# CWBudde/go-pocket-tts

Measured on AMD Instinct MI355X. Metric: synthesized audio sec/sec (xRT), higher is better.
Workload: dtype bf16; 1 GPU; b64_10s_bf16: 64 utterances/GPU x 125 frames (10.0 s each), 25-token prompt + 125-frame voice state, greedy (temperature 0), hipGraph-captured AR step, Mimi decode to 24 kHz PCM written to host; batch_per_gpu=64, frames=125, weights=BF16, kv=bf16, checkpoint=synthetic, shapes of tts_b6369a24 (seed 1234)

## Files before the change

go-pocket-tts_amd/csrc/flow_cluster.hip:

```cpp
#include <hip/hip_ext.h>

#include "../../include/ptts.h"
#include "common.h"
#include "kernels.h"
#include "device_util.h"

namespace ptts {

typedef __bf16 fc_bf16x8 __attribute__((ext_vector_type(8)));
typedef __bf16 fc_bf16x2 __attribute__((ext_vector_type(2)));
typedef float fc_f32x2 __attribute__((ext_vector_type(2)));
typedef float fc_f32x4 __attribute__((ext_vector_type(4)));
typedef unsigned fc_u32x4 __attribute__((ext_vector_type(4)));

constexpr int FC_C = 512;
constexpr int FC_RB = 2048, FC_CMASK = 127;
constexpr unsigned FC_SPIN_LIMIT = 1u << 15;
constexpr int FC_FAULT_WORD = 32 * kFlowClusterMaxTiles;

union FcFrag {
    fc_bf16x8 v;
    uint4 q;
};

__device__ __forceinline__ void fc_split2(float a, float b, unsigned& hi, unsigned& lo) {
    fc_f32x2 f = {a, b};
    fc_bf16x2 h = __builtin_convertvector(f, fc_bf16x2);
    fc_f32x2 r = f - __builtin_convertvector(h, fc_f32x2);
    fc_bf16x2 l = __builtin_convertvector(r, fc_bf16x2);
    hi = *reinterpret_cast<unsigned*>(&h);
    lo = *reinterpret_cast<unsigned*>(&l);
}

__device__ __forceinline__ void fc_stage(unsigned char* Xh, unsigned char* Xl, int wave, int lane, const float4 (&xr)[2]) {
#pragma unroll
    for (int j = 0; j < 2; j++) {
        const int k = (lane + 64 * j) * 4;
        unsigned h01, l01, h23, l23;
// ... 8 lines not shown
template <typename RS>
__device__ __forceinline__ bool fc_sweep(RS rs, int row_off, int lane, unsigned tag, float4 (&xr)[2]) {
    fc_u32x4 g0 = {0u, 0u, 0u, 0u}, g1 = g0, g2 = g0, g3 = g0;
    bool got = true;
    const int voff = row_off + lane * 32;
    const int watch = row_off + ((lane >> 1) * 16 + 6 + 8 * (lane & 1)) * 8;
    for (unsigned spins = 0;; spins++) {
        asm volatile("" ::: "memory");
        const fc_u32x4 w = __builtin_amdgcn_raw_buffer_load_b128(rs, watch, 0, 16);
        if (__all(w[1] == tag && w[3] == tag)) {
            asm volatile("" ::: "memory");
            g0 = __builtin_amdgcn_raw_buffer_load_b128(rs, voff, 0, 16);
            g1 = __builtin_amdgcn_raw_buffer_load_b128(rs, voff + 16, 0, 16);
            g2 = __builtin_amdgcn_raw_buffer_load_b128(rs, voff + 2048, 0, 16);
            g3 = __builtin_amdgcn_raw_buffer_load_b128(rs, voff + 2064, 0, 16);
            const bool ok = g0[1] == tag && g0[3] == tag && g1[1] == tag && g1[3] == tag && g2[1] == tag && g2[3] == tag && g3[1] == tag && g3[3] == tag;
            if (__all(ok)) break;
        }
        if (spins > FC_SPIN_LIMIT) { got = false; g0 = g1 = g2 = g3 = fc_u32x4{0u, 0u, 0u, 0u}; break; }
        __builtin_amdgcn_s_sleep(8);
    }
    xr[0] = make_float4(__uint_as_float(g0[0]), __uint_as_float(g0[2]), __uint_as_float(g1[0]), __uint_as_float(g1[2]));
    xr[1] = make_float4(__uint_as_float(g2[0]), __uint_as_float(g2[2]), __uint_as_float(g3[0]), __uint_as_float(g3[2]));
    return got;
}

template <typename RS>
__device__ __forceinline__ void fc_publish(RS rs, int voff, unsigned tag, const float (&v)[4]) {
    const fc_u32x4 a = {__float_as_uint(v[0]), tag, __float_as_uint(v[1]), tag}, b = {__float_as_uint(v[2]), tag, __float_as_uint(v[3]), tag};
    __builtin_amdgcn_raw_buffer_store_b128(a, rs, voff, 0, 16);
    __builtin_amdgcn_raw_buffer_store_b128(b, rs, voff + 16, 0, 16);
}

constexpr int FC_ROWS = kFlowClusterRows;
constexpr int FC_THREADS = 64 * (4 + FC_ROWS);
constexpr int FC_TILE_GRANULES = 2 * 16 * FC_C;

template <bool STAMP>
__global__ __launch_bounds__(FC_THREADS) void k_flow_cluster(FlowClusterArgs a) {
#define FC_STAMP(i) do { if (STAMP && lane == 0) a.stamps[blockIdx.x * 64 + (i)] = __builtin_amdgcn_s_memrealtime(); } while (0)
    __shared__ __attribute__((aligned(16))) unsigned char Xh[16 * FC_RB];
    __shared__ __attribute__((aligned(16))) unsigned char Xl[16 * FC_RB];
    const int tid = threadIdx.x, lane = tid & 63, wave = __builtin_amdgcn_readfirstlane(tid >> 6);
    const int cb = blockIdx.x & 7, tile = blockIdx.x >> 3;
    const int m0 = tile * FC_ROWS;
    unsigned* const sync = a.sync + tile * 32;
    const unsigned base = __builtin_amdgcn_readfirstlane(__hip_atomic_load(sync, __ATOMIC_RELAXED, __HIP_MEMORY_SCOPE_AGENT));
    auto rs = __builtin_amdgcn_make_buffer_rsrc(a.xbuf + (size_t)tile * FC_TILE_GRANULES, 0, FC_TILE_GRANULES * 8, 0x00020000);
    constexpr int BUF1 = 16 * FC_C * 8;

    if (wave < 4) {
        const int cg = wave, q = lane >> 4, i16 = lane & 15;
        const bool s_ok = i16 < FC_ROWS && m0 + i16 < a.rows;
        const int64_t srow = s_ok ? m0 + i16 : 0;
        const int scol = cb * 64 + cg * 16 + q * 4;
        const int pub_off = i16 * (FC_C * 8) + scol * 8;
        const int64_t wfrag = ((int64_t)(cb * 4 + cg) * 16) * 64 + lane;
        uint4 w[16];
        {
            const uint4* s0 = reinterpret_cast<const uint4*>(a.w0[0]) + wfrag;
#pragma unroll
            for (int i = 0; i < 16; i++) w[i] = s0[i * 64];
        }
        float4 res = *reinterpret_cast<const float4*>(a.fx_in + srow * FC_C + scol);
        auto product = [&](float (&acc)[4]) {
#pragma unroll
            for (int ss = 0; ss < 4; ss++) {
                fc_f32x4 acc_h = {0.f, 0.f, 0.f, 0.f}, acc_l = {0.f, 0.f, 0.f, 0.f};
#pragma unroll
                for (int s = 0; s < 4; s++) {
                    const int off = i16 * FC_RB + (((q * 4 + s) ^ i16) << 4) + ss * 256;
                    FcFrag xh, xl, wv;
                    xh.q = *reinterpret_cast<const uint4*>(&Xh[off]);
                    xl.q = *reinterpret_cast<const uint4*>(&Xl[off]);
                    wv.q = w[ss * 4 + s];
                    acc_h = __builtin_amdgcn_mfma_f32_16x16x32_bf16(wv.v, xh.v, acc_h, 0, 0, 0);
                    acc_l = __builtin_amdgcn_mfma_f32_16x16x32_bf16(wv.v, xl.v, acc_l, 0, 0, 0);
                }
                const fc_f32x4 accv = acc_h + acc_l;
                if (ss == 0) { acc[0] = accv[0]; acc[1] = accv[1]; acc[2] = accv[2]; acc[3] = accv[3]; }
                else { acc[0] += accv[0]; acc[1] += accv[1]; acc[2] += accv[2]; acc[3] += accv[3]; }
            }
        };
        auto next_weights = [&](const void* wt) {
            const uint4* sw = reinterpret_cast<const uint4*>(wt) + wfrag;
#pragma unroll
            for (int i = 0; i < 16; i++) w[i] = sw[i * 64];
        };
        if (wave == 0) FC_STAMP(0);
#pragma unroll 1
        for (int r = 0; r < a.depth; r++) {
            const int rn = min(r + 1, a.depth - 1);
            const void* const pw2 = a.w2[r]; const void* const pw0n = a.w0[rn];
            const float* const pb0 = a.b0[r]; const float* const pb2 = a.b2[r];
            asm volatile("" ::"s"(pw2), "s"(pw0n), "s"(pb0), "s"(pb2));
            const float4 bias0 = *reinterpret_cast<const float4*>(pb0 + scol);
            float acc[4];
            __syncthreads();
            if (wave == 0) FC_STAMP(1 + 4 * r);
            product(acc);
            next_weights(pw2);
            if (STAMP && wave == 0 && r == 2) { if (acc[0] == 1.2345e-30f) FC_STAMP(60); FC_STAMP(56); }
            {
                const float h[4] = {silu1(acc[0] + bias0.x), silu1(acc[1] + bias0.y), silu1(acc[2] + bias0.z), silu1(acc[3] + bias0.w)};
                if (STAMP && wave == 0 && r == 2) { if (h[0] == 1.2345e-30f) FC_STAMP(60); FC_STAMP(58); }
                if (s_ok && !(a.inject && tile == 0 && cb == 7 && r == a.inject - 1)) fc_publish(rs, BUF1 + pub_off, base + 2 * r + 1, h);
            }
            if (STAMP && wave == 0 && r == 2) FC_STAMP(57);
            if (wave == 0) FC_STAMP(2 + 4 * r);
            const float4 bias2 = *reinterpret_cast<const float4*>(pb2 + scol);
            const float4 gate = *reinterpret_cast<const float4*>(a.ada + srow * a.ldmod + (int64_t)(r * 3 + 2) * FC_C + scol);
            __syncthreads();
            if (wave == 0) FC_STAMP(3 + 4 * r);
            product(acc);
            next_weights(pw0n);
            res.x = res.x + gate.x * (acc[0] + bias2.x);
            res.y = res.y + gate.y * (acc[1] + bias2.y);
            res.z = res.z + gate.z * (acc[2] + bias2.z);
            res.w = res.w + gate.w * (acc[3] + bias2.w);
            if (s_ok) {
                if (r + 1 < a.depth) {
                    const float v[4] = {res.x, res.y, res.z, res.w};
                    fc_publish(rs, pub_off, base + 2 * r + 2, v);
                } else *reinterpret_cast<float4*>(a.fx_out + srow * FC_C + scol) = res;
            }
            if (wave == 0) FC_STAMP(4 + 4 * r);
        }
        if (cb == 0 && tid == 0) __hip_atomic_store(sync, base + 2u * (unsigned)a.depth, __ATOMIC_RELAXED, __HIP_MEMORY_SCOPE_AGENT);
        if (wave == 0) FC_STAMP(31);
    } else {
        const int row = wave - 4;
        const bool row_ok = m0 + row < a.rows;
        const int64_t mrow = row_ok ? m0 + row : 0;
        const int kc0 = lane * 4, kc1 = (lane + 64) * 4;
        const int sweep_off = row * (FC_C * 8);
        unsigned fault = 0;
#pragma unroll 1
        for (int r = 0; r < a.depth; r++) {
            if (row_ok) {
                float4 xr[2];
                const float* lnw = a.ln_w[r]; const float* lnb = a.ln_b[r];
                const float* shift = a.ada + mrow * a.ldmod + (int64_t)(r * 3) * FC_C; const float* scale = shift + FC_C;
                const float4 lw0 = *reinterpret_cast<const float4*>(lnw + kc0), lw1 = *reinterpret_cast<const float4*>(lnw + kc1);
                const float4 lb0 = *reinterpret_cast<const float4*>(lnb + kc0), lb1 = *reinterpret_cast<const float4*>(lnb + kc1);
                const float4 lc0 = *reinterpret_cast<const float4*>(scale + kc0), lc1 = *reinterpret_cast<const float4*>(scale + kc1);
                const float4 lh0 = *reinterpret_cast<const float4*>(shift + kc0), lh1 = *reinterpret_cast<const float4*>(shift + kc1);
                if (r == 0) {
                    xr[0] = *reinterpret_cast<const float4*>(a.fx_in + mrow * FC_C + kc0);
                    xr[1] = *reinterpret_cast<const float4*>(a.fx_in + mrow * FC_C + kc1);
                } else if (!fc_sweep(rs, sweep_off, lane, base + 2 * r, xr)) fault = 1;
                if (wave == 4) FC_STAMP(32 + 4 * r);
                fc_f32x2 s2 = {0.f, 0.f};
#pragma unroll
                for (int j = 0; j < 2; j++) s2 += fc_f32x2{xr[j].x, xr[j].z} + fc_f32x2{xr[j].y, xr[j].w};
                const float rk = __builtin_amdgcn_rcpf((float)FC_C);
                const float mean = wave_sum_dpp(s2.x + s2.y) * rk;
                const fc_f32x2 m2 = {mean, mean};
                fc_f32x2 v2 = {0.f, 0.f};
#pragma unroll
                for (int j = 0; j < 2; j++) {
                    const fc_f32x2 da = fc_f32x2{xr[j].x, xr[j].y} - m2, db = fc_f32x2{xr[j].z, xr[j].w} - m2;
                    v2 += da * da + db * db;
                }
                const float inv_std = __builtin_amdgcn_rsqf(wave_sum_dpp(v2.x + v2.y) * rk + a.eps[r]);
                const fc_f32x2 is2 = {inv_std, inv_std};
#pragma unroll
                for (int j = 0; j < 2; j++) {
                    const float4 lw = j ? lw1 : lw0, lb = j ? lb1 : lb0, lc = j ? lc1 : lc0, lh = j ? lh1 : lh0;
                    fc_f32x2 oa = (fc_f32x2{xr[j].x, xr[j].y} - m2) * is2, ob = (fc_f32x2{xr[j].z, xr[j].w} - m2) * is2;
                    oa = oa * fc_f32x2{lw.x, lw.y} + fc_f32x2{lb.x, lb.y};
                    ob = ob * fc_f32x2{lw.z, lw.w} + fc_f32x2{lb.z, lb.w};
                    const fc_f32x2 one = {1.0f, 1.0f};
                    oa = oa * (fc_f32x2{lc.x, lc.y} + one) + fc_f32x2{lh.x, lh.y};
                    ob = ob * (fc_f32x2{lc.z, lc.w} + one) + fc_f32x2{lh.z, lh.w};
                    xr[j] = make_float4(oa.x, oa.y, ob.x, ob.y);
                }
                fc_stage(Xh, Xl, row, lane, xr);
            }
            if (wave == 4) FC_STAMP(33 + 4 * r);
            __syncthreads();
            if (row_ok) {
                float4 xr[2];
                if (!fc_sweep(rs, BUF1 + sweep_off, lane, base + 2 * r + 1, xr)) fault = 1;
                if (wave == 4) FC_STAMP(34 + 4 * r);
                fc_stage(Xh, Xl, row, lane, xr);
            }
            if (wave == 4) FC_STAMP(35 + 4 * r);
            __syncthreads();
        }
        if (fault && lane == 0) atomicOr(a.sync + FC_FAULT_WORD, 1u);
    }
#undef FC_STAMP
}

bool flow_cluster_supported(const FlowClusterArgs& a, int C) {
    if (C != FC_C || a.rows <= 0 || a.rows > kFlowClusterMaxTiles * kFlowClusterRows || a.depth <= 0 || a.depth > FC_MAX_DEPTH || a.ldmod % 4 != 0 || !a.xbuf || !a.sync) return false;
    if (!aligned16(a.fx_in) || !aligned16(a.fx_out) || !aligned16(a.ada)) return false;
    for (int r = 0; r < a.depth; r++)
        if (!a.w0[r] || !a.w2[r] || !a.b0[r] || !a.b2[r] || !a.ln_w[r] || !a.ln_b[r] || !aligned16(a.b0[r]) || !aligned16(a.b2[r]) || !aligned16(a.ln_w[r]) || !aligned16(a.ln_b[r])) return false;
    return true;
}

bool flow_cluster_fits(int rows, int device) {
    int cus = 0, per_cu = 0;
    if (hipDeviceGetAttribute(&cus, hipDeviceAttributeMultiprocessorCount, device) != hipSuccess || cus <= 0) return false;
    if (hipOccupancyMaxActiveBlocksPerMultiprocessor(&per_cu, k_flow_cluster<false>, FC_THREADS, 0) != hipSuccess || per_cu <= 0) { (void)hipGetLastError(); return false; }
    return 8 * ((rows + FC_ROWS - 1) / FC_ROWS) <= cus * per_cu;
}

void launch_flow_cluster(const FlowClusterArgs& a, hipStream_t stream, hipEvent_t ev0, hipEvent_t ev1) {
    note_launch("k_flow_cluster");
    const dim3 grid(8 * ((a.rows + FC_ROWS - 1) / FC_ROWS));
    if (a.stamps) hipLaunchKernelGGL(k_flow_cluster<true>, grid, dim3(FC_THREADS), 0, stream, a);
    else if (ev0) hipExtLaunchKernelGGL(k_flow_cluster<false>, grid, dim3(FC_THREADS), 0, stream, ev0, ev1, 0, a);
    else hipLaunchKernelGGL(k_flow_cluster<false>, grid, dim3(FC_THREADS), 0, stream, a);
}

}
```

go-pocket-tts_amd/csrc/kernels.h:

```cpp
#pragma once

#include <hip/hip_runtime.h>
#include <atomic>
#include <cstdint>
#include <map>
#include <string>
#include <vector>

namespace ptts {

struct RowMap {
    int64_t ld = 0;
    int64_t rows_per_batch = 0;
    int64_t batch_stride = 0;
};

enum AOp : int { AOP_NONE = 0, AOP_ELU = 1 };
enum Epi : int {
    EPI_NONE = 0,
    EPI_GELU,
    EPI_SILU,
    EPI_ELU,
    EPI_RESADD,
    EPI_SCALE_RESADD,
// ... 264 lines not shown
};
struct RowLinArgs {
    const float* x = nullptr; RowMap xmap;
    const float* ln_w = nullptr; const float* ln_b = nullptr; float eps = 1e-5f;
    const void* img = nullptr;
    float* y = nullptr; RowMap ymap;
    const float* rope_cos = nullptr; const float* rope_sin = nullptr; int rope_cols = 0, rope_pos0 = 0, rope_rows_per_seg = 0;
    int M = 0, N = 0, K = 0;
};
bool mimi_rowlin_supported(const RowLinArgs& a);
void launch_mimi_rowlin(const RowLinArgs& a, hipStream_t stream);
bool mimi_ffn_supported(const FfnArgs& a);
void launch_mimi_ffn(const FfnArgs& a, hipStream_t stream);

constexpr int FC_MAX_DEPTH = 8;
struct FlowClusterArgs {
    const float* fx_in = nullptr; float* fx_out = nullptr;
    const float* ada = nullptr; int64_t ldmod = 0;
    int rows = 0, depth = 0;
    float eps[FC_MAX_DEPTH] = {};
    const float* ln_w[FC_MAX_DEPTH] = {}; const float* ln_b[FC_MAX_DEPTH] = {};
    const void* w0[FC_MAX_DEPTH] = {}; const float* b0[FC_MAX_DEPTH] = {};
    const void* w2[FC_MAX_DEPTH] = {}; const float* b2[FC_MAX_DEPTH] = {};
    unsigned long long* xbuf = nullptr;
    unsigned long long* stamps = nullptr;
    int inject = 0;
    unsigned* sync = nullptr;
};
constexpr int kFlowClusterRows = 12;
constexpr int kFlowClusterMaxTiles = (kStepMaxRows + kFlowClusterRows - 1) / kFlowClusterRows;
constexpr size_t kFlowClusterTileBytes = (size_t)2 * 16 * 512 * 8;
constexpr size_t kFlowClusterSyncBytes = (size_t)(32 * kFlowClusterMaxTiles + 32) * 4;
inline size_t flow_cluster_xbuf_bytes(int rows) { return (size_t)((rows + kFlowClusterRows - 1) / kFlowClusterRows) * kFlowClusterTileBytes; }
bool flow_cluster_fits(int rows, int device);
bool flow_cluster_supported(const FlowClusterArgs& a, int C);
void launch_flow_cluster(const FlowClusterArgs& a, hipStream_t stream, hipEvent_t ev0 = nullptr, hipEvent_t ev1 = nullptr);

struct StepState {
    int32_t* kv_len;
    int32_t* active;
    int32_t* step;
    int32_t* countdown;
    int32_t* n_frames;
    int32_t* eos_step;
    int32_t* max_steps;
    int32_t* frames_after_eos;
    float*   eos_threshold;
    int32_t* n_active;
    int32_t* broke;
};
struct StepChain {
    const void* w_in; const float* b_in; float* x; int32_t d_in;
    const void* w_pj; const float* b_pj; float* fx; int32_t d_pj;
    const float* bos; float* x0; int32_t w_bf16; int32_t ok;
};
struct StepFinish {
    StepState s;
    const float* eos_logit;
    float* latents;
    int64_t lat_stride;
    int32_t ldim;
    StepChain ch;
};
struct StepOpenLinears {
    const void* w_in = nullptr; const float* b_in = nullptr; int d_in = 0; float* x = nullptr;
    const void* w_pj = nullptr; const float* b_pj = nullptr; int d_pj = 0; float* fx = nullptr;
    int w_bf16 = 0;
};
bool step_open_mfma_ok(const StepOpenLinears& lin, int ldim);
void launch_step_begin(const StepState& s, const float* latents, int64_t lat_stride, const float* bos, const float* noise, int64_t noise_stride,
                       int ldim, int b, float* in32, float* x0, const StepOpenLinears* lin, hipStream_t stream);
void launch_step_finish(const StepState& s, const float* frame, const float* eos_logit, int ldim, int b, float* latents,
                        int64_t lat_stride, hipStream_t stream);
struct NoiseSpec { uint64_t seed; float sigma; int32_t rows; };
void launch_noise_fill(const NoiseSpec* spec_dev, int n_slots, int max_rows, float* out, int64_t out_stride, int ldim, hipStream_t stream);
struct GatherTable { struct Row { int32_t src_row, dst_off, nf, T; }; Row rows[128]; };
void launch_gather_frames(const GatherTable& t, int n, const float* stage, int64_t row_stride, float* dst, int ld, hipStream_t stream);
void launch_readback_i32(const int32_t* a, int na, const int32_t* b, int nb, int32_t* host, hipStream_t stream);
struct SlotAdmit { int32_t slot, max_steps, frames_after_eos; float eos_threshold; int32_t kv_len, pre_len; const void* pre_k; const void* pre_v; };
void launch_slot_admit(const StepState& s, int32_t* pre_len, const void** pre_k, const void** pre_v, const SlotAdmit* dev, int n, hipStream_t stream);
void launch_slot_retire(const StepState& s, const int32_t* slots_dev, int n, hipStream_t stream);
void launch_fill_i32(int32_t* p, int32_t v, int n, hipStream_t stream);
void launch_add_i32(int32_t* p, const int32_t* inc, int n, hipStream_t stream);

void launch_enc_head(const float* pcm, const void* w, int w_bf16, const float* b, int64_t L, int C, int k, float* out, int64_t ldo, hipStream_t stream);
int enc_ds_splits(int M, int N, int K);
void launch_enc_downsample(const float* A, int64_t lda, const void* W, int w_bf16, const float* bias, int M, int N, int K, float* partial, float* out,
                           hipStream_t stream);

void launch_bct_to_btc(const float* in, int b, int c, int t, float* out, int out_pad_rows, hipStream_t stream);
void launch_btc_to_bct(const float* in, int in_pad_rows, int b, int c, int t, float* out, hipStream_t stream);

}
```

go-pocket-tts_amd/csrc/runtime.cpp:

```cpp
#include "runtime.h"

#include <chrono>

#include <algorithm>
#include <cmath>

namespace ptts {

static RowMap flat(int64_t ld) { return RowMap{ld, 0, 0}; }
static RowMap seg(int64_t ld, int64_t rows_per_batch, int64_t batch_stride) { return RowMap{ld, rows_per_batch, batch_stride}; }

static GemmArgs mk(const Model& m, const float* A, RowMap am, const Lin& l, float* C, RowMap cm, int M) {
    GemmArgs g;
    g.A = A; g.amap = am;
    g.W = m.arena + l.w; g.w_bf16 = l.bf16; g.ldw = l.in;
    g.Wt = l.wt == NONE ? nullptr : m.arena + l.wt;
    g.wt_i8 = l.wt_i8; g.wscale = m.at<float>(l.wscale);
    g.bias = m.at<float>(l.b);
    g.C = C; g.cmap = cm;
    g.M = M; g.N = l.out; g.K = l.in;
    return g;
}
static LnArgs mkln(const Model& m, const float* x, RowMap xm, const Norm& n, float* y, int64_t ldy, int rows) {
    LnArgs a;
// ... 219 lines not shown
    b->vcache.ensure(kvbytes);
    PTTS_HIP(hipMemsetAsync(b->kcache.p, 0, kvbytes, m.stream));
    PTTS_HIP(hipMemsetAsync(b->vcache.p, 0, kvbytes, m.stream));
    b->state_i32.ensure((9 * B + 1) * sizeof(int32_t));
    b->state_f32.ensure(B * sizeof(float));
    int32_t* s = b->state_i32.as<int32_t>();
    b->st.kv_len = s; b->st.active = s + B; b->st.step = s + 2 * B; b->st.countdown = s + 3 * B;
    b->st.n_frames = s + 4 * B; b->st.eos_step = s + 5 * B; b->st.max_steps = s + 6 * B;
    b->st.frames_after_eos = s + 7 * B; b->st.broke = s + 8 * B; b->st.n_active = s + 9 * B;
    b->st.eos_threshold = b->state_f32.as<float>();
    b->kv_len_host.assign(B, 0);
    b->pre_k.ensure((size_t)B * sizeof(void*)); b->pre_v.ensure((size_t)B * sizeof(void*)); b->pre_len.ensure((size_t)B * sizeof(int32_t));
    b->pre_k_host.assign(B, nullptr); b->pre_v_host.assign(B, nullptr); b->pre_len_host.assign(B, 0);
    const size_t f = sizeof(float);
    const int NA = d.ada_all.out;
    b->in_raw.ensure(B * d.ldim * f); b->in32.ensure(B * d.ldim * f);
    b->x.ensure(B * d.d_model * f); b->xn.ensure(B * std::max(d.d_model, d.flow_dim) * f);
    b->qkv.ensure(B * 3 * d.d_model * f); b->attn.ensure(B * d.d_model * f);
    b->ff.ensure(B * d.ffn * f); b->last.ensure(B * d.d_model * f); b->eos.ensure(B * f);
    b->sy.ensure(B * d.flow_dim * f); b->ada.ensure(B * NA * f);
    b->fx.ensure(B * d.flow_dim * f); b->fh.ensure(B * d.flow_dim * f); b->fh2.ensure(B * d.flow_dim * f);
    b->cur.ensure(B * d.ldim * f);
    b->partial.ensure((size_t)16 * B * std::max(d.d_model, d.flow_dim) * f);
    b->latents.ensure(B * b->max_steps * d.ldim * f);
    {
        StepFinish sf{b->st, b->eos.as<float>(), b->latents.as<float>(), (int64_t)b->max_steps * d.ldim, (int32_t)d.ldim, StepChain{}};
        StepOpenLinears lin;
        b->chain_ok = open_linears(*b, lin) && step_open_mfma_ok(lin, d.ldim) && ((int64_t)b->max_steps * d.ldim) % 2 == 0 &&
                      (lin.w_bf16 != 0) == (d.final_linear.bf16 != 0 || d.final_linear.wt_i8 != 0);
        b->fx2.ensure(B * d.flow_dim * f); b->cur2.ensure(B * d.ldim * f);
        StepFinish sf2[2] = {sf, sf};
        sf2[0].ch = StepChain{lin.w_in, lin.b_in, lin.x, lin.d_in, lin.w_pj, lin.b_pj, b->fx2.as<float>(), lin.d_pj, m.at<float>(d.bos), b->cur2.as<float>(), lin.w_bf16, b->chain_ok ? 1 : 0};
        sf2[1].ch = StepChain{lin.w_in, lin.b_in, lin.x, lin.d_in, lin.w_pj, lin.b_pj, b->fx.as<float>(), lin.d_pj, m.at<float>(d.bos), b->cur.as<float>(), lin.w_bf16, b->chain_ok ? 1 : 0};
        b->fin_dev.ensure(sizeof sf2);
        h2d(b->fin_dev.p, sf2, sizeof sf2, m.stream);
    }
    {
        const char* sw = getenv("PTTS_FLOW_CLUSTER");
        const bool off = sw && sw[0] == '0';
        bool ok = !off && !m.fc_disabled.load() && d.flow_dim == 512 && d.flow_depth > 0 && d.flow_depth <= FC_MAX_DEPTH && n_slots <= kStepMaxRows &&
                  flow_cluster_fits(n_slots, m.device);
        for (int r = 0; ok && r < d.flow_depth; r++) {
            const auto& rb = d.rb[r];
            for (const Lin* l : {&rb.mlp0, &rb.mlp2}) ok = ok && l->in == 512 && l->out == 512 && l->bf16 && !l->wt_i8 && l->wt != NONE && l->b != NONE;
            ok = ok && rb.ln.w != NONE && rb.ln.b != NONE && rb.ln.d == 512;
        }
        b->fc_ok = ok;
        if (ok) {
            b->fc_xbuf.ensure(flow_cluster_xbuf_bytes(n_slots)); b->fc_sync.ensure(kFlowClusterSyncBytes);
            PTTS_HIP(hipMemsetAsync(b->fc_xbuf.p, 0, flow_cluster_xbuf_bytes(n_slots), m.stream));
            PTTS_HIP(hipMemsetAsync(b->fc_sync.p, 0, kFlowClusterSyncBytes, m.stream));
            if (getenv("PTTS_FC_STAMPS")) { b->fc_stamps.ensure((size_t)8 * kFlowClusterMaxTiles * 64 * 8); PTTS_HIP(hipMemsetAsync(b->fc_stamps.p, 0, (size_t)8 * kFlowClusterMaxTiles * 64 * 8, m.stream)); }
        }
    }
    {
        const char* sw = getenv("PTTS_TALL");
        bool ok = !(sw && sw[0] == '0') && n_slots >= kTallMinRows && (d.d_model == 512 || d.d_model == 1024) && d.ffn % 128 == 0;
        for (int l = 0; ok && l < d.n_layers; l++) {
            const auto& L = d.layers[l];
            for (const Lin* li : {&L.in_proj, &L.l1, &L.l2}) ok = ok && li->bf16 && !li->wt_i8 && li->wt != NONE && li->out % 4 == 0;
            ok = ok && L.in_proj.in == d.d_model && L.l1.in == d.d_model && L.l1.out == d.ffn && L.l2.in == d.ffn && L.l2.out == d.d_model;
            ok = ok && L.n1.w != NONE && L.n1.b != NONE && L.n2.w != NONE && L.n2.b != NONE;
        }
        b->tall_ok = ok;
        if (ok) { b->tp_a.ensure(2 * B * d.d_model * sizeof(uint16_t)); b->tp_f.ensure(2 * B * d.ffn * sizeof(uint16_t)); }
    }
    PTTS_HIP(hipHostMalloc((void**)&b->n_active_pinned, sizeof(int32_t) * (size_t)(2 + 2 * B), hipHostMallocDefault));
    PTTS_HIP(hipHostMalloc((void**)&b->rows_pinned, sizeof(PcmRow) * std::max<size_t>((size_t)B, 1), hipHostMallocDefault));
    batch_reset(*b);
    return b.release();
}

void batch_reset(Batch& b) {
    b.opened = false;
    hipStream_t s = b.m->stream;
    const int B = b.B;
    launch_fill_i32(b.st.kv_len, 0, B, s);
    b.kv_bound = 0;
    launch_fill_i32(b.st.active, 1, B, s);
    launch_fill_i32(b.st.step, 0, B, s);
// ... 300 lines not shown
    ln.x = x; ln.xmap = flat(l.in); ln.eps = in.eps; ln.rows = M; ln.d = l.in;
    if (in.norm && in.affine) { ln.w = m.at<float>(in.norm->w); ln.b = m.at<float>(in.norm->b); }
    ln.shift = in.shift; ln.scale = in.scale; ln.ldmod = in.ldmod;
    ln.partial = in.pend.partial; ln.splitk = in.pend.splitk; ln.pstride = in.pend.pstride; ln.pbias = in.pend.bias;
    float* y = in.y_out ? in.y_out : b.xn.as<float>();
    ln.y = y; ln.ldy = l.in;
    if (in.pend.partial) {
        launch_layernorm(ln, m.stream);
        if (in.x_out && in.x_out != x) PTTS_HIP(hipMemcpyAsync(in.x_out, x, (size_t)M * l.in * sizeof(float), hipMemcpyDeviceToDevice, m.stream));
    } else launch_layernorm(ln, m.stream);
    GemmArgs g2 = mk(m, y, flat(l.in), l, C, flat(ldc), M);
    g2.epi = epi; g2.addvec = addvec; g2.R = R; g2.alpha = alpha;
    step_gemm(m, g2);
    return false;
}

static bool open_linears(Batch& b, StepOpenLinears& lin) {
    Model& m = *b.m;
    const Desc& d = m.d;
    const int ld = d.ldim;
    if (!(ld <= 64 && ld % 4 == 0 && d.input_linear.in == ld && d.input_proj.in == ld && d.input_linear.bf16 == d.input_proj.bf16)) return false;
    lin.w_in = m.arena + d.input_linear.w; lin.b_in = m.at<float>(d.input_linear.b); lin.d_in = d.input_linear.out; lin.x = b.x.as<float>();
    lin.w_pj = m.arena + d.input_proj.w; lin.b_pj = m.at<float>(d.input_proj.b); lin.d_pj = d.input_proj.out; lin.fx = b.fx.as<float>();
    lin.w_bf16 = d.input_linear.bf16;
    return true;
}

void flow_cluster_recover(Batch& b) {
    hipStream_t s = b.m->stream;
    (void)hipStreamSynchronize(s);
    (void)hipMemsetAsync(b.fc_xbuf.p, 0, flow_cluster_xbuf_bytes(b.B), s);
    (void)hipMemsetAsync(b.fc_sync.p, 0, kFlowClusterSyncBytes, s);
    (void)hipStreamSynchronize(s);
    b.fc_ok = false;
    for (auto& set : b.graphs) for (auto& row : set) for (hipGraphExec_t& g : row) if (g) { (void)hipGraphExecDestroy(g); g = nullptr; }
    for (auto& gs : b.graph_steps) gs[0] = gs[1] = 0;
    b.opened = false;
    b.m->fc_disabled.store(true);
    b.m->fc_fallbacks.fetch_add(1);
}
void flow_cluster_fault(Batch& b) {
    flow_cluster_recover(b);
    throw FlowClusterFault(PTTS_ENODEVICE, "ptts-hip: the flow net's in-launch hand-off timed out (k_flow_cluster); the steps concerned are re-issued as launches");
}

void step_open(Batch& b) {
    Model& m = *b.m;
    const Desc& d = m.d;
    const int ld = d.ldim;
    const int64_t ls = (int64_t)b.max_steps * ld;
    StepOpenLinears lin;
    const bool ok = open_linears(b, lin);
    b.opened = ok;
    b.par = 0;
    launch_step_begin(b.st, b.latents.as<float>(), ls, m.at<float>(d.bos), b.has_noise ? b.noise.as<float>() : nullptr, ls, ld, b.B,
                      b.in32.as<float>(), b.cur.as<float>(), ok ? &lin : nullptr, m.stream);
}

bool step_core(Batch& b, int lsd, bool opened, bool fuse_finish, bool chain) {
    bool finished = false;
    b.opened = false;
    if (!opened) b.par = 0;
    Model& m = *b.m;
    const Desc& d = m.d;
    hipStream_t s = m.stream;
    const int B = b.B, D = d.d_model, C = d.flow_dim;
    const bool kvb = m.opts.kv == PTTS_KV_BF16;
// ... 127 lines not shown
            ln.partial = pend.partial; ln.splitk = pend.splitk; ln.pstride = pend.pstride; ln.pbias = pend.bias;
            launch_layernorm(ln, s);
            step_gemm(m, mk(m, last, flat(D), d.out_eos, b.eos.as<float>(), flat(1), B));
        }
    }
    b.tail_fused = tail_fused;
    finished = step_flow(b, lsd, opened, fuse_finish, chain);
    if (!b.capturing) b.kv_bound++;
    return finished;
}

static bool step_flow(Batch& b, int lsd, bool opened, bool fuse_finish, bool chain) {
    bool finished = false;
    Model& m = *b.m;
    const Desc& d = m.d;
    const int B = b.B, D = d.d_model, C = d.flow_dim, NA = d.ada_all.out;
    hipStream_t s = m.stream;
    const bool tail_fused = b.tail_fused;
    float* last = b.last.as<float>();
    float* sy = b.sy.as<float>();
    const float* tc = m.tcomb.at(lsd)->as<float>();
    float* ada = b.ada.as<float>();
    float* fx = b.fx_now();
    float* fh2 = b.fh2.as<float>();
    float* cur = b.cur_now();
    for (int i = 0; i < lsd; i++) {
        if (i > 0 || !tail_fused) {
            GemmArgs gc = mk(m, last, flat(D), d.cond_embed, sy, flat(C), B);
            gc.epi = EPI_SILU; gc.addvec = tc + (size_t)i * C;
            step_gemm(m, gc);
        }
        step_gemm(m, mk(m, sy, flat(C), d.ada_all, ada, flat(NA), B));
        if (i > 0 || !opened) step_gemm(m, mk(m, cur, flat(d.ldim), d.input_proj, fx, flat(C), B));
        bool clustered = false;
        if (b.fc_ok) {
            FlowClusterArgs fa;
            fa.fx_in = fx; fa.fx_out = fx; fa.ada = ada; fa.ldmod = NA; fa.rows = B; fa.depth = d.flow_depth;
            for (int r = 0; r < d.flow_depth; r++) {
                const auto& rb = d.rb[r];
                fa.eps[r] = rb.ln.eps; fa.ln_w[r] = m.at<float>(rb.ln.w); fa.ln_b[r] = m.at<float>(rb.ln.b);
                fa.w0[r] = m.arena + rb.mlp0.wt; fa.b0[r] = m.at<float>(rb.mlp0.b);
                fa.w2[r] = m.arena + rb.mlp2.wt; fa.b2[r] = m.at<float>(rb.mlp2.b);
            }
            fa.xbuf = b.fc_xbuf.as<unsigned long long>(); fa.sync = b.fc_sync.as<unsigned>();
            if (b.fc_stamps.p) fa.stamps = b.fc_stamps.as<unsigned long long>();
            if (m.fc_inject && !b.capturing) { fa.inject = m.fc_inject; m.fc_inject = 0; }
            if (flow_cluster_supported(fa, C)) {
                launch_flow_cluster(fa, s);
                clustered = true;
            }
        }
        for (int r = 0; !clustered && r < d.flow_depth; r++) {
            const auto& rb = d.rb[r];
            FusedIn in;
            in.norm = &rb.ln; in.eps = rb.ln.eps;
            in.shift = ada + (size_t)r * 3 * C; in.scale = in.shift + C; in.ldmod = NA;
            step_fused_linear(b, fx, in, rb.mlp0, fh2, C, B, EPI_SILU, nullptr, nullptr, 1.0f);
            GemmArgs g2 = mk(m, fh2, flat(C), rb.mlp2, fx, flat(C), B);
            g2.R = fx; g2.epi = EPI_GATE_RESADD; g2.gate = ada + (size_t)r * 3 * C + 2 * C; g2.ldg = NA;
            step_gemm(m, g2);
        }
        FusedIn fin;
        fin.affine = false; fin.eps = 1e-6f;
        fin.shift = ada + (size_t)d.flow_depth * 3 * C; fin.scale = fin.shift + C; fin.ldmod = NA;
        if (fuse_finish && i == lsd - 1) {
            fin.finish = b.fin_dev.as<StepFinish>() + b.par;
            if (chain && b.chain_ok) {
                fin.chain = true;
                fin.chain_noise = b.has_noise ? b.noise.as<float>() : nullptr;
                fin.chain_noise_stride = (int64_t)b.max_steps * d.ldim;
            }
        }
        bool chained = false;
        finished = step_fused_linear(b, fx, fin, d.final_linear, cur, d.ldim, B, EPI_AXPY, nullptr, cur, 1.0f / (float)lsd, nullptr, &chained);
        if (chained) { b.opened = true; b.par ^= 1; }
    }
    return finished;
}

void step_flow_again(Batch& b, int lsd) {
    b.opened = false; b.par = 0;
    (void)step_flow(b, lsd, false, false, false);
}

void mimi_setup(Model& m, MimiWs& w, int B, int T) {
    const Desc& d = m.d;
    w.B = B; w.T = T;
    const int C = d.mimi_dim, S = d.up_stride, T1 = T * S, F = d.mimi_ffn;
    w.P0 = d.init_k - 1;
    w.Ls[0] = T1; w.Ps[0] = 1;
    for (int j = 0; j < 3; j++) {
        w.Ls[j + 1] = w.Ls[j] * d.strides[j];
        int need_next = j < 2 ? 1 : d.final_k - 1;
// ... 933 lines not shown
```

go-pocket-tts_amd/csrc/runtime.h:

```cpp
#pragma once

#include <atomic>
#include <functional>

#include "kernels.h"
#include "model.h"
#include "row_ring.h"
#include "dsp_spec.h"
#include "host_rows.h"

namespace ptts {

struct DevBuf {
    void* p = nullptr;
    size_t n = 0;
    DevBuf() = default;
    DevBuf(const DevBuf&) = delete;
    DevBuf& operator=(const DevBuf&) = delete;
    ~DevBuf() { release(); }
    void release() {
        if (p) (void)hipFree(p);
        p = nullptr;
        n = 0;
    }
// ... 96 lines not shown
struct PackedRows {
    std::vector<size_t> bytes, off;
    char* base = nullptr;
    PackedRows(Model& m, WorkSlot slot, std::vector<size_t> row_bytes, const bool* skip = nullptr) : bytes(std::move(row_bytes)), off(bytes.size()) {
        base = m.work(slot, std::max<size_t>(pack_rows(bytes.data(), skip, (int)bytes.size(), off.data()), kRowAlign)).as<char>();
    }
    char* row(int i) const { return base + off[(size_t)i]; }
    void upload(int i, const void* src, hipStream_t s) const { PTTS_HIP(hipMemcpyAsync(row(i), src, bytes[(size_t)i], hipMemcpyHostToDevice, s)); }
    void download(int i, void* dst, hipStream_t s) const { PTTS_HIP(hipMemcpyAsync(dst, row(i), bytes[(size_t)i], hipMemcpyDeviceToHost, s)); }
};

struct Batch {
    Model* m = nullptr;
    int B = 0;
    int cap = 0;
    int max_steps = 0;
    DevBuf kcache, vcache;
    DevBuf state_i32;
    DevBuf state_f32;
    StepState st{};
    std::vector<int32_t> kv_len_host;
    DevBuf pre_k, pre_v, pre_len;
    std::vector<const void*> pre_k_host, pre_v_host;
    std::vector<int32_t> pre_len_host;
    DevBuf in_raw, in32, x, xn, qkv, attn, ff, last, eos, sy, ada, fx, fh, fh2, cur, noise_step, partial;
    DevBuf latents;
    DevBuf noise;
    bool has_noise = false;
    bool opened = false;
    bool chain_ok = false;
    DevBuf fx2, cur2;
    DevBuf fc_xbuf, fc_sync, fc_stamps;
    bool fc_ok = false;
    DevBuf tp_a, tp_f;
    bool tall_ok = false;
    bool tail_fused = false;
    unsigned* fc_fault() const { return fc_sync.as<unsigned>() + 32 * kFlowClusterMaxTiles; }
    int par = 0;
    float* fx_now() const { return (par ? fx2 : fx).as<float>(); }
    float* cur_now() const { return (par ? cur2 : cur).as<float>(); }
    hipStream_t io_stream = nullptr;
    bool slot_local = false;
    int kv_bound = 0;
    bool capturing = false;
    hipGraphExec_t graphs[2][17][3] = {};
    int graph_steps[2][2] = {{0, 0}, {0, 0}};
    int graph_lsd = 0;
    int capture_keys = 0;
    int32_t* n_active_pinned = nullptr;
    PcmRow* rows_pinned = nullptr;
    DevBuf fin_dev;

    ~Batch();
    size_t kv_elem() const { return m->opts.kv == PTTS_KV_BF16 ? 2 : 4; }
    void* kc(int layer) const { return (char*)kcache.p + (size_t)layer * B * m->d.heads * cap * m->d.hd * kv_elem(); }
    void* vc(int layer) const { return (char*)vcache.p + (size_t)layer * B * m->d.heads * cap * m->d.hd * kv_elem(); }
};

void* result_alloc(size_t bytes);
void result_free(void* p);
bool result_is_pinned(const void* p);

struct Voice {
    Model* m = nullptr;
    int device = 0;
    int offset = 0;
// ... 187 lines not shown
```

Measured before the change: 12790 x real-time.

## Fuse flow final linear, step finish, and next-step open into flow cluster kernel

On the last flow sub-step, the persistent flow-cluster kernel now also runs the final LayerNorm, the final linear with the Euler AXPY update, latent write-out, the EOS/step-state update, and the chained input/projection linears for the next AR step. Before, these ran as a separate fused-linear launch after the cluster kernel. The goal is to remove that launch and its global round trip of fx from the captured per-step graph. In exchange the kernel uses more shared memory and registers (which may lower occupancy) and its control logic becomes considerably more complex; it can be disabled with PTTS_FLOW_TAIL=0.

```diff
diff --git a/go-pocket-tts_amd/csrc/flow_cluster.hip b/go-pocket-tts_amd/csrc/flow_cluster.hip
--- a/go-pocket-tts_amd/csrc/flow_cluster.hip
+++ b/go-pocket-tts_amd/csrc/flow_cluster.hip
@@ -4,6 +4,9 @@
 #include "common.h"
 #include "kernels.h"
 #include "device_util.h"
+#include "step_open.h"
+
+#include <type_traits>
 
 namespace ptts {
 
@@ -78,12 +81,48 @@
     __builtin_amdgcn_raw_buffer_store_b128(b, rs, voff + 16, 0, 16);
 }
 
+template <bool AFFINE>
+__device__ __forceinline__ void fc_norm(float4 (&xr)[2], float eps, const float4& lw0, const float4& lw1, const float4& lb0, const float4& lb1, const float4& lc0,
+                                        const float4& lc1, const float4& lh0, const float4& lh1) {
+    fc_f32x2 s2 = {0.f, 0.f};
+#pragma unroll
+    for (int j = 0; j < 2; j++) s2 += fc_f32x2{xr[j].x, xr[j].z} + fc_f32x2{xr[j].y, xr[j].w};
+    const float rk = __builtin_amdgcn_rcpf((float)FC_C);
+    const float mean = wave_sum_dpp(s2.x + s2.y) * rk;
+    const fc_f32x2 m2 = {mean, mean};
+    fc_f32x2 v2 = {0.f, 0.f};
+#pragma unroll
+    for (int j = 0; j < 2; j++) {
+        const fc_f32x2 da = fc_f32x2{xr[j].x, xr[j].y} - m2, db = fc_f32x2{xr[j].z, xr[j].w} - m2;
+        v2 += da * da + db * db;
+    }
+    const float inv_std = __builtin_amdgcn_rsqf(wave_sum_dpp(v2.x + v2.y) * rk + eps);
+    const fc_f32x2 is2 = {inv_std, inv_std};
+#pragma unroll
+    for (int j = 0; j < 2; j++) {
+        const float4 lc = j ? lc1 : lc0, lh = j ? lh1 : lh0;
+        fc_f32x2 oa = (fc_f32x2{xr[j].x, xr[j].y} - m2) * is2, ob = (fc_f32x2{xr[j].z, xr[j].w} - m2) * is2;
+        if constexpr (AFFINE) {
+            const float4 lw = j ? lw1 : lw0, lb = j ? lb1 : lb0;
+            oa = oa * fc_f32x2{lw.x, lw.y} + fc_f32x2{lb.x, lb.y};
+            ob = ob * fc_f32x2{lw.z, lw.w} + fc_f32x2{lb.z, lb.w};
+        }
+        const fc_f32x2 one = {1.0f, 1.0f};
+        oa = oa * (fc_f32x2{lc.x, lc.y} + one) + fc_f32x2{lh.x, lh.y};
+        ob = ob * (fc_f32x2{lc.z, lc.w} + one) + fc_f32x2{lh.z, lh.w};
+        xr[j] = make_float4(oa.x, oa.y, ob.x, ob.y);
+    }
+}
+
 constexpr int FC_ROWS = kFlowClusterRows;
 constexpr int FC_THREADS = 64 * (4 + FC_ROWS);
 constexpr int FC_TILE_GRANULES = 2 * 16 * FC_C;
 
-template <bool STAMP>
-__global__ __launch_bounds__(FC_THREADS) void k_flow_cluster(FlowClusterArgs a) {
+struct FcNoTail {};
+constexpr int FC_X_GROUPS = 7 * FC_ROWS;
+
+template <bool STAMP, bool TAIL>
+__global__ __launch_bounds__(FC_THREADS) void k_flow_cluster(FlowClusterArgs a, std::conditional_t<TAIL, FlowClusterTail, FcNoTail> t) {
 #define FC_STAMP(i) do { if (STAMP && lane == 0) a.stamps[blockIdx.x * 64 + (i)] = __builtin_amdgcn_s_memrealtime(); } while (0)
     __shared__ __attribute__((aligned(16))) unsigned char Xh[16 * FC_RB];
     __shared__ __attribute__((aligned(16))) unsigned char Xl[16 * FC_RB];
@@ -94,6 +133,8 @@
     const unsigned base = __builtin_amdgcn_readfirstlane(__hip_atomic_load(sync, __ATOMIC_RELAXED, __HIP_MEMORY_SCOPE_AGENT));
     auto rs = __builtin_amdgcn_make_buffer_rsrc(a.xbuf + (size_t)tile * FC_TILE_GRANULES, 0, FC_TILE_GRANULES * 8, 0x00020000);
     constexpr int BUF1 = 16 * FC_C * 8;
+    __shared__ __attribute__((aligned(16))) unsigned char planes[TAIL ? 4 * 16 * SO_PITCH : 16];
+    [[maybe_unused]] unsigned char* const fh = planes, * const fl = planes + 16 * SO_PITCH, * const nh = planes + 32 * SO_PITCH, * const nl = planes + 48 * SO_PITCH;
 
     if (wave < 4) {
         const int cg = wave, q = lane >> 4, i16 = lane & 15;
@@ -137,7 +178,12 @@
 #pragma unroll 1
         for (int r = 0; r < a.depth; r++) {
             const int rn = min(r + 1, a.depth - 1);
-            const void* const pw2 = a.w2[r]; const void* const pw0n = a.w0[rn];
+            [[maybe_unused]] const bool last = r + 1 == a.depth;
+            const void* pw0n = a.w0[rn];
+            if constexpr (TAIL) {
+                if (last) pw0n = reinterpret_cast<const uint4*>(t.wf) + ((int64_t)((cg & 1) - (cb * 4 + cg)) * 16) * 64;
+            }
+            const void* const pw2 = a.w2[r];
             const float* const pb0 = a.b0[r]; const float* const pb2 = a.b2[r];
             asm volatile("" ::"s"(pw2), "s"(pw0n), "s"(pb0), "s"(pb2));
             const float4 bias0 = *reinterpret_cast<const float4*>(pb0 + scol);
@@ -165,12 +211,60 @@
             res.z = res.z + gate.z * (acc[2] + bias2.z);
             res.w = res.w + gate.w * (acc[3] + bias2.w);
             if (s_ok) {
-                if (r + 1 < a.depth) {
+                if (TAIL || r + 1 < a.depth) {
                     const float v[4] = {res.x, res.y, res.z, res.w};
                     fc_publish(rs, pub_off, base + 2 * r + 2, v);
                 } else *reinterpret_cast<float4*>(a.fx_out + srow * FC_C + scol) = res;
             }
             if (wave == 0) FC_STAMP(4 + 4 * r);
+        }
+        if constexpr (TAIL) {
+            const int fcol = (cg & 1) * 16 + q * 4;
+            const float4 t_bias = *reinterpret_cast<const float4*>(t.bf + fcol);
+            const float4 t_er = *reinterpret_cast<const float4*>(t.cur + srow * SO_K + fcol);
+            const float4 t_bos = *reinterpret_cast<const float4*>(t.fin.ch.bos + fcol);
+            int f_act = 0, f_step = 0, f_cd = 0, f_fae = 0, f_max = 0, f_kv = 0;
+            float f_logit = 0.f, f_thr = 0.f;
+            if (cb == 0) {
+                const StepState& fs = t.fin.s;
+                f_act = fs.active[srow]; f_step = fs.step[srow]; f_cd = fs.countdown[srow]; f_fae = fs.frames_after_eos[srow];
+                f_max = fs.max_steps[srow]; f_kv = fs.kv_len[srow]; f_logit = t.fin.eos_logit[srow]; f_thr = fs.eos_threshold[srow];
+            }
+            __syncthreads();
+            if (cg < 2) {
+                float acc[4];
+                product(acc);
+                const float bias[4] = {t_bias.x, t_bias.y, t_bias.z, t_bias.w}, er[4] = {t_er.x, t_er.y, t_er.z, t_er.w}, bos[4] = {t_bos.x, t_bos.y, t_bos.z, t_bos.w};
+                float v[4];
+#pragma unroll
+                for (int reg = 0; reg < 4; reg++) v[reg] = acc[reg] + bias[reg];
+#pragma unroll
+                for (int reg = 0; reg < 4; reg++) v[reg] = er[reg] + t.alpha * v[reg];
+#pragma unroll
+                for (int reg = 0; reg < 4; reg++) so_put(fh, fl, i16, fcol + reg, isnan(v[reg]) ? bos[reg] : v[reg]);
+                if (cb == 0 && s_ok && f_act) {
+                    *reinterpret_cast<float4*>(t.fin.latents + srow * t.fin.lat_stride + (int64_t)f_step * t.fin.ldim + fcol) = make_float4(v[0], v[1], v[2], v[3]);
+                    if (cg == 0 && q == 0) {
+                        const StepState& fs = t.fin.s;
+                        const int st = f_step;
+                        const bool is_eos = f_logit > f_thr;
+                        int cd = f_cd;
+                        bool done = false;
+                        if (is_eos && cd < 0) { cd = f_fae; fs.eos_step[srow] = st; }
+                        if (cd >= 0) {
+                            if (cd == 0) { done = true; fs.broke[srow] = 1; }
+                            else cd--;
+                        }
+                        fs.countdown[srow] = cd;
+                        fs.n_frames[srow] = st + 1;
+                        fs.step[srow] = st + 1;
+                        fs.kv_len[srow] = f_kv + 1;
+                        if (st + 1 >= f_max) done = true;
+                        if (done) { fs.active[srow] = 0; atomicSub(fs.n_active, 1); }
+                    }
+                }
+            }
+            __syncthreads();
         }
         if (cb == 0 && tid == 0) __hip_atomic_store(sync, base + 2u * (unsigned)a.depth, __ATOMIC_RELAXED, __HIP_MEMORY_SCOPE_AGENT);
         if (wave == 0) FC_STAMP(31);
@@ -196,31 +290,7 @@
                     xr[1] = *reinterpret_cast<const float4*>(a.fx_in + mrow * FC_C + kc1);
                 } else if (!fc_sweep(rs, sweep_off, lane, base + 2 * r, xr)) fault = 1;
                 if (wave == 4) FC_STAMP(32 + 4 * r);
-                fc_f32x2 s2 = {0.f, 0.f};
-#pragma unroll
-                for (int j = 0; j < 2; j++) s2 += fc_f32x2{xr[j].x, xr[j].z} + fc_f32x2{xr[j].y, xr[j].w};
-                const float rk = __builtin_amdgcn_rcpf((float)FC_C);
-                const float mean = wave_sum_dpp(s2.x + s2.y) * rk;
-                const fc_f32x2 m2 = {mean, mean};
-                fc_f32x2 v2 = {0.f, 0.f};
-#pragma unroll
-                for (int j = 0; j < 2; j++) {
-                    const fc_f32x2 da = fc_f32x2{xr[j].x, xr[j].y} - m2, db = fc_f32x2{xr[j].z, xr[j].w} - m2;
-                    v2 += da * da + db * db;
-                }
-                const float inv_std = __builtin_amdgcn_rsqf(wave_sum_dpp(v2.x + v2.y) * rk + a.eps[r]);
-                const fc_f32x2 is2 = {inv_std, inv_std};
-#pragma unroll
-                for (int j = 0; j < 2; j++) {
-                    const float4 lw = j ? lw1 : lw0, lb = j ? lb1 : lb0, lc = j ? lc1 : lc0, lh = j ? lh1 : lh0;
-                    fc_f32x2 oa = (fc_f32x2{xr[j].x, xr[j].y} - m2) * is2, ob = (fc_f32x2{xr[j].z, xr[j].w} - m2) * is2;
-                    oa = oa * fc_f32x2{lw.x, lw.y} + fc_f32x2{lb.x, lb.y};
-                    ob = ob * fc_f32x2{lw.z, lw.w} + fc_f32x2{lb.z, lb.w};
-                    const fc_f32x2 one = {1.0f, 1.0f};
-                    oa = oa * (fc_f32x2{lc.x, lc.y} + one) + fc_f32x2{lh.x, lh.y};
-                    ob = ob * (fc_f32x2{lc.z, lc.w} + one) + fc_f32x2{lh.z, lh.w};
-                    xr[j] = make_float4(oa.x, oa.y, ob.x, ob.y);
-                }
+                fc_norm<true>(xr, a.eps[r], lw0, lw1, lb0, lb1, lc0, lc1, lh0, lh1);
                 fc_stage(Xh, Xl, row, lane, xr);
             }
             if (wave == 4) FC_STAMP(33 + 4 * r);
@@ -233,6 +303,50 @@
             }
             if (wave == 4) FC_STAMP(35 + 4 * r);
             __syncthreads();
+        }
+        if constexpr (TAIL) {
+            float4 lc0, lc1, lh0, lh1;
+            float2 vs = make_float2(0.f, 0.f);
+            if (row_ok) {
+                const float* shift = a.ada + mrow * a.ldmod + (int64_t)(a.depth * 3) * FC_C; const float* scale = shift + FC_C;
+                lc0 = *reinterpret_cast<const float4*>(scale + kc0); lc1 = *reinterpret_cast<const float4*>(scale + kc1);
+                lh0 = *reinterpret_cast<const float4*>(shift + kc0); lh1 = *reinterpret_cast<const float4*>(shift + kc1);
+                if (cb == 0 && lane < 16 && t.noise) {
+                    const StepState& fs = t.fin.s;
+                    const int c_st = fs.step[mrow], c_max = fs.max_steps[mrow], c_act = fs.active[mrow];
+                    if (c_act && c_st + 1 < c_max) vs = *reinterpret_cast<const float2*>(t.noise + mrow * t.noise_stride + (int64_t)(c_st + 1) * SO_K + lane * 2);
+                }
+            }
+            const StepChain& ch = t.fin.ch;
+            const bool c_fx = cb == 0;
+            const void* const c_wp = c_fx ? ch.w_pj : ch.w_in; const float* const c_bp = c_fx ? ch.b_pj : ch.b_in;
+            float* const c_out = c_fx ? ch.fx : ch.x;
+            const int c_n = c_fx ? ch.d_pj : ch.d_in, c_t0 = c_fx ? row : row * 7 + (cb - 1), c_stride = c_fx ? FC_ROWS : FC_X_GROUPS;
+            constexpr int CT = 3;
+            SoW<true> cw[CT];
+#pragma unroll
+            for (int i = 0; i < CT; i++) cw[i] = so_load_w<true>(c_wp, c_bp, min((c_t0 + i * c_stride) * 16, c_n - 16), c_n, lane);
+            if (row_ok) {
+                float4 xr[2];
+                if (!fc_sweep(rs, sweep_off, lane, base + 2 * a.depth, xr)) fault = 1;
+                fc_norm<false>(xr, t.eps, lc0, lc1, lc0, lc1, lc0, lc1, lh0, lh1);
+                fc_stage(Xh, Xl, row, lane, xr);
+            }
+            __syncthreads();
+            if (cb == 0 && lane < 16) {
+                so_put(nh, nl, row, lane * 2, vs.x);
+                so_put(nh, nl, row, lane * 2 + 1, vs.y);
+            }
+            __syncthreads();
+            if (cb == 0 && lane < 16 && row_ok) *reinterpret_cast<float2*>(ch.x0 + mrow * SO_K + lane * 2) = vs;
+            const unsigned char* const ph = c_fx ? nh : fh, * const pl = c_fx ? nl : fl;
+            const int m_end = min(a.rows, m0 + FC_ROWS);
+            for (int i = 0;; i++) {
+                const int n0 = (c_t0 + i * c_stride) * 16;
+                if (n0 >= c_n) break;
+                const SoW<true> w = i == 0 ? cw[0] : i == 1 ? cw[1] : i == 2 ? cw[2] : so_load_w<true>(c_wp, c_bp, n0, c_n, lane);
+                so_tile<true>(ph, pl, w, n0, c_out, c_n, m0, m_end, lane);
+            }
         }
         if (fault && lane == 0) atomicOr(a.sync + FC_FAULT_WORD, 1u);
     }
@@ -247,19 +361,34 @@
     return true;
 }
 
-bool flow_cluster_fits(int rows, int device) {
+bool flow_cluster_tail_supported(const FlowClusterArgs& a, const FlowClusterTail& t) {
+    const StepChain& ch = t.fin.ch;
+    return ch.ok && ch.w_bf16 && t.fin.ldim == SO_K && t.fin.lat_stride % 4 == 0 && aligned16(t.fin.latents) && t.wf && t.bf && aligned16(t.bf) && t.cur && aligned16(t.cur) &&
+           aligned16(ch.bos) && ch.d_in > 0 && ch.d_in % 16 == 0 && ch.d_pj > 0 && ch.d_pj % 16 == 0 && ch.x && ch.fx && ch.x0 && aligned16(ch.x) && aligned16(ch.fx) && aligned16(ch.x0) &&
+           ch.x0 != t.cur && ch.fx != a.fx_in && (!t.noise || t.noise_stride % 2 == 0) && a.ada != nullptr;
+}
+
+bool flow_cluster_fits(int rows, int device, bool tail) {
     int cus = 0, per_cu = 0;
     if (hipDeviceGetAttribute(&cus, hipDeviceAttributeMultiprocessorCount, device) != hipSuccess || cus <= 0) return false;
-    if (hipOccupancyMaxActiveBlocksPerMultiprocessor(&per_cu, k_flow_cluster<false>, FC_THREADS, 0) != hipSuccess || per_cu <= 0) { (void)hipGetLastError(); return false; }
+    const hipError_t e = tail ? hipOccupancyMaxActiveBlocksPerMultiprocessor(&per_cu, k_flow_cluster<false, true>, FC_THREADS, 0)
+                              : hipOccupancyMaxActiveBlocksPerMultiprocessor(&per_cu, k_flow_cluster<false, false>, FC_THREADS, 0);
+    if (e != hipSuccess || per_cu <= 0) { (void)hipGetLastError(); return false; }
     return 8 * ((rows + FC_ROWS - 1) / FC_ROWS) <= cus * per_cu;
 }
 
-void launch_flow_cluster(const FlowClusterArgs& a, hipStream_t stream, hipEvent_t ev0, hipEvent_t ev1) {
+void launch_flow_cluster(const FlowClusterArgs& a, hipStream_t stream, hipEvent_t ev0, hipEvent_t ev1, const FlowClusterTail* tail) {
     note_launch("k_flow_cluster");
     const dim3 grid(8 * ((a.rows + FC_ROWS - 1) / FC_ROWS));
-    if (a.stamps) hipLaunchKernelGGL(k_flow_cluster<true>, grid, dim3(FC_THREADS), 0, stream, a);
-    else if (ev0) hipExtLaunchKernelGGL(k_flow_cluster<false>, grid, dim3(FC_THREADS), 0, stream, ev0, ev1, 0, a);
-    else hipLaunchKernelGGL(k_flow_cluster<false>, grid, dim3(FC_THREADS), 0, stream, a);
-}
-
-}
+    if (tail) {
+        note_launch("k_flow_cluster+tail");
+        if (ev0) hipExtLaunchKernelGGL((k_flow_cluster<false, true>), grid, dim3(FC_THREADS), 0, stream, ev0, ev1, 0, a, *tail);
+        else hipLaunchKernelGGL((k_flow_cluster<false, true>), grid, dim3(FC_THREADS), 0, stream, a, *tail);
+        return;
+    }
+    if (a.stamps) hipLaunchKernelGGL((k_flow_cluster<true, false>), grid, dim3(FC_THREADS), 0, stream, a, FcNoTail{});
+    else if (ev0) hipExtLaunchKernelGGL((k_flow_cluster<false, false>), grid, dim3(FC_THREADS), 0, stream, ev0, ev1, 0, a, FcNoTail{});
+    else hipLaunchKernelGGL((k_flow_cluster<false, false>), grid, dim3(FC_THREADS), 0, stream, a, FcNoTail{});
+}
+
+}
diff --git a/go-pocket-tts_amd/csrc/kernels.h b/go-pocket-tts_amd/csrc/kernels.h
--- a/go-pocket-tts_amd/csrc/kernels.h
+++ b/go-pocket-tts_amd/csrc/kernels.h
@@ -320,9 +320,10 @@
 constexpr size_t kFlowClusterTileBytes = (size_t)2 * 16 * 512 * 8;
 constexpr size_t kFlowClusterSyncBytes = (size_t)(32 * kFlowClusterMaxTiles + 32) * 4;
 inline size_t flow_cluster_xbuf_bytes(int rows) { return (size_t)((rows + kFlowClusterRows - 1) / kFlowClusterRows) * kFlowClusterTileBytes; }
-bool flow_cluster_fits(int rows, int device);
+bool flow_cluster_fits(int rows, int device, bool tail = false);
 bool flow_cluster_supported(const FlowClusterArgs& a, int C);
-void launch_flow_cluster(const FlowClusterArgs& a, hipStream_t stream, hipEvent_t ev0 = nullptr, hipEvent_t ev1 = nullptr);
+struct FlowClusterTail;
+void launch_flow_cluster(const FlowClusterArgs& a, hipStream_t stream, hipEvent_t ev0 = nullptr, hipEvent_t ev1 = nullptr, const FlowClusterTail* tail = nullptr);
 
 struct StepState {
     int32_t* kv_len;
@@ -350,6 +351,14 @@
     int32_t ldim;
     StepChain ch;
 };
+struct FlowClusterTail {
+    StepFinish fin;
+    const void* wf = nullptr; const float* bf = nullptr;
+    const float* cur = nullptr;
+    float alpha = 1.0f, eps = 1e-6f;
+    const float* noise = nullptr; int64_t noise_stride = 0;
+};
+bool flow_cluster_tail_supported(const FlowClusterArgs& a, const FlowClusterTail& t);
 struct StepOpenLinears {
     const void* w_in = nullptr; const float* b_in = nullptr; int d_in = 0; float* x = nullptr;
     const void* w_pj = nullptr; const float* b_pj = nullptr; int d_pj = 0; float* fx = nullptr;
diff --git a/go-pocket-tts_amd/csrc/runtime.cpp b/go-pocket-tts_amd/csrc/runtime.cpp
--- a/go-pocket-tts_amd/csrc/runtime.cpp
+++ b/go-pocket-tts_amd/csrc/runtime.cpp
@@ -275,6 +275,7 @@
         StepFinish sf2[2] = {sf, sf};
         sf2[0].ch = StepChain{lin.w_in, lin.b_in, lin.x, lin.d_in, lin.w_pj, lin.b_pj, b->fx2.as<float>(), lin.d_pj, m.at<float>(d.bos), b->cur2.as<float>(), lin.w_bf16, b->chain_ok ? 1 : 0};
         sf2[1].ch = StepChain{lin.w_in, lin.b_in, lin.x, lin.d_in, lin.w_pj, lin.b_pj, b->fx.as<float>(), lin.d_pj, m.at<float>(d.bos), b->cur.as<float>(), lin.w_bf16, b->chain_ok ? 1 : 0};
+        b->fin_host[0] = sf2[0]; b->fin_host[1] = sf2[1];
         b->fin_dev.ensure(sizeof sf2);
         h2d(b->fin_dev.p, sf2, sizeof sf2, m.stream);
     }
@@ -289,6 +290,12 @@
             ok = ok && rb.ln.w != NONE && rb.ln.b != NONE && rb.ln.d == 512;
         }
         b->fc_ok = ok;
+        {
+            const char* tw = getenv("PTTS_FLOW_TAIL");
+            const Lin& fl = d.final_linear;
+            b->fc_tail = ok && !(tw && tw[0] == '0') && b->chain_ok && d.ldim == 32 && fl.in == 512 && fl.out == d.ldim && fl.bf16 && !fl.wt_i8 && fl.wt != NONE && fl.b != NONE &&
+                         d.input_linear.bf16 && flow_cluster_fits(n_slots, m.device, true);
+        }
         if (ok) {
             b->fc_xbuf.ensure(flow_cluster_xbuf_bytes(n_slots)); b->fc_sync.ensure(kFlowClusterSyncBytes);
             PTTS_HIP(hipMemsetAsync(b->fc_xbuf.p, 0, flow_cluster_xbuf_bytes(n_slots), m.stream));
@@ -655,7 +662,7 @@
     (void)hipMemsetAsync(b.fc_xbuf.p, 0, flow_cluster_xbuf_bytes(b.B), s);
     (void)hipMemsetAsync(b.fc_sync.p, 0, kFlowClusterSyncBytes, s);
     (void)hipStreamSynchronize(s);
-    b.fc_ok = false;
+    b.fc_ok = false; b.fc_tail = false;
     for (auto& set : b.graphs) for (auto& row : set) for (hipGraphExec_t& g : row) if (g) { (void)hipGraphExecDestroy(g); g = nullptr; }
     for (auto& gs : b.graph_steps) gs[0] = gs[1] = 0;
     b.opened = false;
@@ -849,7 +856,7 @@
         }
         step_gemm(m, mk(m, sy, flat(C), d.ada_all, ada, flat(NA), B));
         if (i > 0 || !opened) step_gemm(m, mk(m, cur, flat(d.ldim), d.input_proj, fx, flat(C), B));
-        bool clustered = false;
+        bool clustered = false, tail_inside = false;
         if (b.fc_ok) {
             FlowClusterArgs fa;
             fa.fx_in = fx; fa.fx_out = fx; fa.ada = ada; fa.ldmod = NA; fa.rows = B; fa.depth = d.flow_depth;
@@ -863,7 +870,15 @@
             if (b.fc_stamps.p) fa.stamps = b.fc_stamps.as<unsigned long long>();
             if (m.fc_inject && !b.capturing) { fa.inject = m.fc_inject; m.fc_inject = 0; }
             if (flow_cluster_supported(fa, C)) {
-                launch_flow_cluster(fa, s);
+                FlowClusterTail ft;
+                if (b.fc_tail && fuse_finish && i == lsd - 1 && chain && b.chain_ok && !fa.stamps) {
+                    ft.fin = b.fin_host[b.par];
+                    ft.wf = m.arena + d.final_linear.wt; ft.bf = m.at<float>(d.final_linear.b);
+                    ft.cur = cur; ft.alpha = 1.0f / (float)lsd; ft.eps = 1e-6f;
+                    ft.noise = b.has_noise ? b.noise.as<float>() : nullptr; ft.noise_stride = (int64_t)b.max_steps * d.ldim;
+                    tail_inside = flow_cluster_tail_supported(fa, ft);
+                }
+                launch_flow_cluster(fa, s, nullptr, nullptr, tail_inside ? &ft : nullptr);
                 clustered = true;
             }
         }
@@ -876,6 +891,11 @@
             GemmArgs g2 = mk(m, fh2, flat(C), rb.mlp2, fx, flat(C), B);
             g2.R = fx; g2.epi = EPI_GATE_RESADD; g2.gate = ada + (size_t)r * 3 * C + 2 * C; g2.ldg = NA;
             step_gemm(m, g2);
+        }
+        if (tail_inside) {
+            finished = true;
+            b.opened = true; b.par ^= 1;
+            break;
         }
         FusedIn fin;
         fin.affine = false; fin.eps = 1e-6f;
diff --git a/go-pocket-tts_amd/csrc/runtime.h b/go-pocket-tts_amd/csrc/runtime.h
--- a/go-pocket-tts_amd/csrc/runtime.h
+++ b/go-pocket-tts_amd/csrc/runtime.h
@@ -152,6 +152,8 @@
     DevBuf fx2, cur2;
     DevBuf fc_xbuf, fc_sync, fc_stamps;
     bool fc_ok = false;
+    bool fc_tail = false;
+    StepFinish fin_host[2] = {};
     DevBuf tp_a, tp_f;
     bool tall_ok = false;
     bool tail_fused = false;
```

Measured after the change: 12790 x real-time. No clear change (-0.0%).
